# MirceaKitsune/python_raytracer

Measured on AMD Instinct MI355X. Metric: Mrays/s (primary+bounce), higher is better.
Workload: dtype f64; 1 GPU; mods/default 3840x2160 spp8 max_bounces8 (BASELINE config 3/4); width=3840, height=2160, samples=8, primary_rays=62725130, bounce_rays=75192856, partition=(x ^ y) % 1, traversed=True, fast_draws=32, frames_in_flight=1, scene_flow=pre-selected camera chunks (fixture), rng_retraced_rays=0, rng_table=static seeds: draw table + ray table built once before the timed region, reused

## Files before the change

### python_raytracer_amd/csrc/vrt_kernels.hip

```cpp
#include <hip/hip_runtime.h>
#include <stdint.h>
#include <stdio.h>
#include <stdlib.h>

#include <mutex>
#include <vector>

#include "../../include/vrt.h"
#include "vrt_math.h"

#pragma clang fp contract(off)

#define VRT_WAVE 64
#define VRT_BLOCK 256

static thread_local int g_last_hip_error = 0;
#define HIP_TRY(expr)                                   \
    do {                                                \
        hipError_t e__ = (expr);                        \
        if (e__ != hipSuccess) {                        \
            g_last_hip_error = (int)e__;                \
            return VRT_ERR_HIP;                         \
        }                                               \
    } while (0)
// ... 711 lines not shown
    unsigned long long* vals;
    unsigned long long* gkeys;
    unsigned long long* gvals;
};
__device__ __forceinline__ unsigned pow_hash(unsigned long long bits) {
    unsigned h = (unsigned)(bits >> 32) * 0x9e3779b1u + (unsigned)bits * 0x85ebca6bu;
    return h >> 24;
}
#define VRT_PW_PROBES 4
#ifndef VRT_POW_INLINE
#define VRT_POW_INLINE __noinline__
#endif
__device__ VRT_POW_INLINE double pow_miss(unsigned long long* keys, unsigned long long* vals, unsigned long long* gkeys,
                                        unsigned long long* gvals, double x, double y) {
    const double v = vrt_pow(x, y);
    const unsigned long long bits = (unsigned long long)__double_as_longlong(x);
    const unsigned long long vb = (unsigned long long)__double_as_longlong(v);
    const unsigned h = pow_hash(bits);
    for (int i = 0; i < VRT_PW_PROBES; i++) {
        const int s = (int)((h + i) & (VRT_PW_SLOTS - 1));
        const unsigned long long old = atomicCAS(&keys[s], 0ull, bits);
        if (old == 0ull || old == bits) {
            __hip_atomic_store(&vals[s], vb, __ATOMIC_RELAXED, __HIP_MEMORY_SCOPE_WORKGROUP);
            break;
        }
    }
    if (gkeys) {
        for (int i = 0; i < VRT_PW_PROBES; i++) {
            const int s = (int)((h + i) & (VRT_PW_SLOTS - 1));
            const unsigned long long old = atomicCAS(&gkeys[s], 0ull, bits);
            if (old == 0ull || old == bits) {
                __hip_atomic_store(&gvals[s], vb, __ATOMIC_RELAXED, __HIP_MEMORY_SCOPE_AGENT);
                break;
            }
        }
    }
    return v;
}
__device__ VRT_POW_INLINE double pow_slow(unsigned long long* keys, unsigned long long* vals, unsigned long long* gkeys,
                                        unsigned long long* gvals, double x, double y) {
    const unsigned long long bits = (unsigned long long)__double_as_longlong(x);
    const unsigned h = pow_hash(bits);
    for (int i = 1; i < VRT_PW_PROBES; i++) {
        const int sidx = (int)((h + i) & (VRT_PW_SLOTS - 1));
        const unsigned long long k = __hip_atomic_load(&keys[sidx], __ATOMIC_RELAXED, __HIP_MEMORY_SCOPE_WORKGROUP);
        if (k == bits) {
            const unsigned long long v = __hip_atomic_load(&vals[sidx], __ATOMIC_RELAXED, __HIP_MEMORY_SCOPE_WORKGROUP);
            if (v != 0ull) return __longlong_as_double((long long)v);
            break;
        }
        if (k == 0ull) break;
    }
    return pow_miss(keys, vals, gkeys, gvals, x, y);
}
__device__ __forceinline__ double pow_cached(const PowCache& pc, double x, double y) {
    if (x == 1.0) return 1.0;
    const unsigned long long bits = (unsigned long long)__double_as_longlong(x);
    const int sidx = (int)pow_hash(bits);
    const unsigned long long k = __hip_atomic_load(&pc.keys[sidx], __ATOMIC_RELAXED, __HIP_MEMORY_SCOPE_WORKGROUP);
    const unsigned long long v = __hip_atomic_load(&pc.vals[sidx], __ATOMIC_RELAXED, __HIP_MEMORY_SCOPE_WORKGROUP);
    if (k == bits && v != 0ull) return __longlong_as_double((long long)v);
    return pow_slow(pc.keys, pc.vals, pc.gkeys, pc.gvals, x, y);
}

__device__ __forceinline__ bool div_safe(double a) {
    const double m = __builtin_fabs(a);
    return m >= 0x1p-500 && m <= 0x1p500;
}
__device__ __forceinline__ double with_sign_of(double mag, double sgn) {
    const unsigned hi = ((unsigned)__double2hiint(mag) & 0x7fffffffu) | ((unsigned)__double2hiint(sgn) & 0x80000000u);
    return __hiloint2double((int)hi, __double2loint(mag));
}
__device__ __forceinline__ void div3_same_divisor(double& a, double& b, double& c, double d) {
    const bool fast = div_safe(d) & ((a == 0.0) | (__builtin_fabs(a) >= 0x1p-500)) & ((b == 0.0) | (__builtin_fabs(b) >= 0x1p-500)) &
                      ((c == 0.0) | (__builtin_fabs(c) >= 0x1p-500));
    if (fast) {
        double y = __builtin_amdgcn_rcp(d);
        double e = __builtin_fma(-d, y, 1.0);
        y = __builtin_fma(y, e, y);
        e = __builtin_fma(-d, y, 1.0);
        y = __builtin_fma(y, e, y);
        double q, r;
        q = a * y; r = __builtin_fma(-d, q, a); a = with_sign_of(__builtin_fma(r, y, q), a);
        q = b * y; r = __builtin_fma(-d, q, b); b = with_sign_of(__builtin_fma(r, y, q), b);
        q = c * y; r = __builtin_fma(-d, q, c); c = with_sign_of(__builtin_fma(r, y, q), c);
    } else {
        a = a / d;
        b = b / d;
        c = c / d;
    }
}

struct Ray {
    double px, py, pz, vx, vy, vz;
    double step, life, bounces, energy;
    int nm4x, nm4y, nm4z;
    uint32_t entry;
    uint32_t boff;
    uint32_t color;
    int ndraw, resnaps;
    uint32_t off;
    uint32_t rowi;
    double d0, d1, d2;
};

__device__ __forceinline__ unsigned long long wave_first_u64(unsigned long long v) {
    const unsigned lo = __builtin_amdgcn_readfirstlane((unsigned)v), hi = __builtin_amdgcn_readfirstlane((unsigned)(v >> 32));
    return ((unsigned long long)hi << 32) | lo;
}

enum { LANE_IDLE = 0, LANE_MARCH = 1, LANE_HIT = 2, LANE_ENDED = 3, LANE_ENDED_BROKE = 4, LANE_ENDED_EXHAUSTED = 5 };
__device__ __forceinline__ int opaque_zero() {
    int z = 0;
    asm volatile("" : "+v"(z));
    return z;
}
enum { COLD_POS = 0, COLD_ROT = 3, COLD_DIST_MIN = 7, COLD_POW_Y, COLD_LOD_BOUNCES, COLD_MAX_LIGHT, COLD_MAX_BOUNCES1,
       COLD_SHUTTER, COLD_CS, COLD_INV_CS, COLD_N };
enum { C_LOOKUP = 0, C_NBR, C_CGET, C_HIT, C_ADV, C_NLOCAL };

typedef __attribute__((address_space(3))) uint32_t lds_u32;
typedef __attribute__((address_space(3))) double lds_f64;
typedef __attribute__((address_space(3))) unsigned long long lds_u64;
typedef __attribute__((address_space(3))) char lds_char;

struct MarchCtx {
    const lds_char* tab;
    int tl[3];
    const lds_u32* ct;
    lds_u32* bm;
    const lds_f64* mats;
    const lds_f64* cold;
    lds_u32* tot;
    PowCache pc;
    __amdgpu_buffer_rsrc_t vox;
    unsigned cs4;
    double cs, inv_cs;
    bool kept_cs;
    bool has_bm, tile;

    int td[3];
    int toc[3], oc[3], dm[3];
    const lds_char* wt;
    int wb[3];
    unsigned cs3;
};
#define COLD(i) C.cold[(i) + opaque_zero()]
enum { CF_HAS_BM = 1, CF_CT_LDS = 2, CF_CT_IDENTITY = 4, CF_HAS_KEYS = 8, CF_BM_WINDOW = 16 };

#ifdef VRT_DIAG
enum { DG_PASSES = 0, DG_CYC_REFILL, DG_CYC_MARCH, DG_CYC_HIT, DG_CYC_END, DG_ITERS, DG_MARCH_LANES, DG_HIT_EXEC,
       DG_HIT_LANES, DG_END_EXEC, DG_END_LANES, DG_REFILL_EXEC, DG_REFILL_LANES, DG_WAVE_CYCLES, DG_SNAP_ITERS,
       DG_SNAP_LANES, DG_BRICK_VISITS, DG_SWAPS, DG_SWAP_LANES, DG_EVICT_LANES, DG_CYC_SWAP, DG_VOID_LANES,
#ifdef VRT_DIAG_HIST
       DG_NV1, DG_H1 = DG_NV1 + 8, DG_N = DG_H1 + 8
#else
       DG_N
#endif
};
__device__ unsigned long long g_diag[DG_N];
__device__ unsigned long long g_diag_t[5];
#define DG_ADD(idx_, val_)                                                                                      \
    do {                                                                                                        \
        const unsigned long long v_ = (unsigned long long)(val_);   \
        const unsigned long long e_ = __ballot(1);                                                              \
        if ((int)(threadIdx.x & 63) == __ffsll((long long)e_) - 1) dg.acc[idx_] += v_;                           \
    } while (0)
#define DG_TIME() __builtin_amdgcn_s_memtime()
struct DgLane {
    __attribute__((address_space(3))) unsigned long long* acc;
    unsigned brick;
    unsigned long long bv;
};
#define DG_BRICK()                                                                                                     \
    do {                                                                                                               \
        const unsigned key_ = (((unsigned)(int)__builtin_floor(r.px) >> 3) & 1023u) |                                  \
                              ((((unsigned)(int)__builtin_floor(r.py) >> 3) & 1023u) << 10) |                          \
                              ((((unsigned)(int)__builtin_floor(r.pz) >> 3) & 1023u) << 20);                           \
        dg.bv += key_ != dg.brick ? 1 : 0;                                                                             \
        dg.brick = key_;                                                                                               \
    } while (0)
#else
struct DgLane {};
#define DG_ADD(i, v)
#define DG_BRICK()
#endif
#ifdef VRT_ISA_MARK
#define VRT_MARK(name) asm volatile("; @@" name)
#else
#define VRT_MARK(name)
#endif

__device__ __forceinline__ void floor3_i32(double x, double y, double z, int& fx, int& fy, int& fz) {
    double a, b, c;
    const double magic = 6755399441055744.0;
    asm volatile(
        "s_setreg_imm32_b32 hwreg(HW_REG_MODE, 2, 2), 2\n\t"
        "v_add_f64 %0, %3, %6\n\t"
        "v_add_f64 %1, %4, %6\n\t"
        "v_add_f64 %2, %5, %6\n\t"
        "s_setreg_imm32_b32 hwreg(HW_REG_MODE, 2, 2), 0"
        : "=&v"(a), "=&v"(b), "=&v"(c)
        : "v"(x), "v"(y), "v"(z), "s"(magic));
    fx = __double2loint(a);
    fy = __double2loint(b);
    fz = __double2loint(c);
}

__device__ __forceinline__ double min3_f64(double a, double b, double c) {
    double t;
    asm("v_min_f64 %0, %1, %2" : "=v"(t) : "v"(a), "v"(b));
    asm("v_min_f64 %0, %1, %2" : "=v"(t) : "v"(t), "v"(c));
    return t;
}
__device__ __forceinline__ double absmax3_f64(double a, double b, double c) {
    double t;
    asm("v_max_f64 %0, |%1|, |%2|" : "=v"(t) : "v"(a), "v"(b));
    asm("v_max_f64 %0, %1, |%2|" : "=v"(t) : "v"(t), "v"(c));
    return t;
}

__device__ __forceinline__ void floor3_i32_lane(double x, double y, double z, double magic, int& fx, int& fy, int& fz) {
    double a, b, c;
    asm volatile(
        "s_setreg_imm32_b32 hwreg(HW_REG_MODE, 2, 2), 2\n\t"
        "v_add_f64 %0, %3, %6\n\t"
        "v_add_f64 %1, %4, %6\n\t"
        "v_add_f64 %2, %5, %6\n\t"
        "s_setreg_imm32_b32 hwreg(HW_REG_MODE, 2, 2), 0"
        : "=&v"(a), "=&v"(b), "=&v"(c)
        : "v"(x), "v"(y), "v"(z), "v"(magic));
    fx = __double2loint(a);
    fy = __double2loint(b);
    fz = __double2loint(c);
}

__device__ __forceinline__ uint32_t tab_at(const MarchCtx& C, int axis, unsigned byte_index) {
    return *reinterpret_cast<const lds_u32*>(C.tab + C.tl[axis] + (int)byte_index);
}

template <int RESMODE>
__device__ __forceinline__ unsigned cell_offset(const MarchCtx& C, uint32_t entry, unsigned base, unsigned m4, unsigned cs4, int nm4x,
                                                int nm4y, int nm4z, int l4x, int l4y, int l4z, bool inside, bool valid) {
    if (RESMODE == 2 && entry >= (3u << 24)) {
        const int3 o = snap_generic3((int)(entry >> 24), -(nm4x >> 2), -(nm4y >> 2), -(nm4z >> 2), l4x >> 2, l4y >> 2, l4z >> 2);
        l4x = o.x << 2;
        l4y = o.y << 2;
        l4z = o.z << 2;
        inside = valid && (unsigned)(l4x | l4y | l4z) < cs4;
        m4 = 0x3fcu;
    }
    if (RESMODE == 0) m4 = ~0u;
    const unsigned t = tab_at(C, 0, (unsigned)l4x & m4) | tab_at(C, 1, (unsigned)l4y & m4) | tab_at(C, 2, (unsigned)l4z & m4);
    return inside ? base + t : ~0u;
}

__device__ __forceinline__ uint32_t finish_color(const PowCache& pc, bool has_background, double pow_y, double shutter, uint32_t color,
                                                 double& energy, double bounces, double vy) {
    int cr = (int)(color & 255u), cg = (int)((color >> 8) & 255u), cb = (int)((color >> 16) & 255u);
    if (has_background) {
        double a = 1 / pow_cached(pc, 1 + bounces, pow_y);
        if (!(a < 1)) a = 1;
        const double up = vy > 0 ? vy : 0;
        const double b2 = 1 - a;
        cr = (int)__builtin_rint((double)cr * b2 + 127.0 * a);
        cg = (int)__builtin_rint((double)cg * b2 + (127 + up * 64) * a);
        cb = (int)__builtin_rint((double)cb * b2 + (127 + up * 128) * a);
        energy = energy * b2 + (1 + up) * a;
        double t;
        t = __builtin_rint((double)cr * energy); cr = t < 255 ? (int)t : 255;
        t = __builtin_rint((double)cg * energy); cg = t < 255 ? (int)t : 255;
        t = __builtin_rint((double)cb * energy); cb = t < 255 ? (int)t : 255;
    }
    double e = energy + shutter;
    if (!(e < 1)) e = 1;
    const int alpha = (int)__builtin_rint(e * 255);
    return (uint32_t)cr | ((uint32_t)cg << 8) | ((uint32_t)cb << 16) | ((uint32_t)alpha << 24);
}

typedef const __attribute__((address_space(4))) MarchParams* kernarg_ptr;
__device__ __forceinline__ const __attribute__((address_space(4))) MarchParams& fresh_args(const MarchParams&) {
    auto p = (kernarg_ptr)__builtin_amdgcn_kernarg_segment_ptr();
    asm volatile("" : "+s"(p));
    return *p;
}


struct LkState {
    uint32_t okey;
    uint64_t oword;
    uint64_t* brick_slot;
};
template <bool RECORD>
struct SeenList {
    int64_t seen[RECORD ? 48 : 1];
    int n;
};

struct PendingVisit {
    int tci;
    int bi;
    uint64_t tkey, tcur;
};

template <bool RECORD, bool TDQ = false, int DEFER = 0, class PT>
__device__ __forceinline__ void resnap_commit(const PT& Q, const MarchCtx& C, Ray& r, int fx, int fy, int fz, uint64_t wmin_key,
// ... 1176 lines not shown
__device__ __forceinline__ uint32_t morton_even_bits(uint32_t v) {
    v &= 0x55555555u;
    v = (v | (v >> 1)) & 0x33333333u;
    v = (v | (v >> 2)) & 0x0f0f0f0fu;
    v = (v | (v >> 4)) & 0x00ff00ffu;
    v = (v | (v >> 8)) & 0x0000ffffu;
    return v;
}
template <class PT>
__device__ __forceinline__ bool tile_ticket(const PT& Q, uint32_t g, int64_t& first_ray) {
    const uint32_t t = g >> Q.tile_px_log2, c = g & ((1u << Q.tile_px_log2) - 1u);
    const uint32_t tx = morton_even_bits(t), ty = morton_even_bits(t >> 1);
    const uint32_t x = (tx << Q.tile_px_log2) + c;
    first_ray = ((int64_t)x * Q.st.height + (int64_t)(ty << Q.tile_px_log2)) * Q.g.smax;
    return x < (uint32_t)Q.st.width && ty < (uint32_t)Q.tile_nty;
}
__device__ __forceinline__ int tile_take(const MarchParams& P, int ts, int lane, int64_t chunk, int64_t& first_ray) {
    const auto& Q = fresh_args(P);
    const uint32_t per_head = 1u << (Q.tile_px_log2 + 2 * Q.tile_log2 - 3);
    first_ray = -1;
    while ((ts & 0x78) != 0x40) {
        uint32_t k = 0;
        if (lane == 0) k = atomicAdd(Q.tile_heads + (ts & 7) * 32, 1u);
        k = (uint32_t)__builtin_amdgcn_readfirstlane((int)k);
        if (k >= per_head) {
            ts = ((ts + 1) & 7) | ((ts & 0x78) + 8) | 0x80;
            continue;
        }
        if ((int64_t)(per_head - k) * chunk < (int64_t)(gridDim.x >> 3) * (2 * VRT_BLOCK)) ts |= 0x80;
        int64_t first;
        if (tile_ticket(Q, (uint32_t)(ts & 7) * per_head + k, first)) {
            first_ray = first;
            break;
        }
    }
    return ts;
}
#define VRT_POOL_STATE_WORD (13 * 2 * VRT_POOL_SLOTS + 9 * VRT_POOL_SLOTS)
#define VRT_POOL_OFF_WORD (13 * 2 * VRT_POOL_SLOTS + 7 * VRT_POOL_SLOTS)

template <int SPEC, int RESMODE, int PERPIX = 0, bool W = false, bool DEFER = false, bool TILE = false>
__global__ void __launch_bounds__(VRT_BLOCK, VRT_WAVES_PER_SIMD) march_pool_kernel(MarchParams P) {
    static_assert(!TILE || DEFER, "tiled hand-out: the instances for scenes beyond the caches");
    static_assert(!W || (RESMODE != 2 && SPEC == 8), "march_step_w");
    static_assert(!(W && DEFER), "deferred key comparison: the shipped march step");
    __shared__ MarchSharedT<W> S;
    extern __shared__ __align__(16) unsigned char s_dyn[];
    MarchCtx C;
    march_prologue<W>(P, S, s_dyn, C);
    const int wave_in_block = threadIdx.x >> 6;
    const int lane = threadIdx.x & 63;
    lds_u64* const pool = (lds_u64*)(s_dyn + P.pool_lds_off + wave_in_block * VRT_POOL_WAVE_BYTES);
    lds_u32* const pool_state = (lds_u32*)pool + VRT_POOL_STATE_WORD;
    if (lane < VRT_POOL_SLOTS) pool_state[lane] = (uint32_t)LANE_IDLE;
    __syncthreads();

    const int64_t count = P.n;
    const int64_t chunk = P.chunk > 0 ? P.chunk : VRT_CHUNK;
    const int64_t tail_start = count - (int64_t)gridDim.x * (2 * VRT_BLOCK);
    int64_t next = 0, range_end = 0;
    bool more = true;
    bool tiled = false;
    int ts = 0;
    if constexpr (TILE) {
        tiled = P.tile_heads != nullptr && P.plan_hdr->full_frame != 0;
        unsigned xcc = 0;
        xcc = __builtin_amdgcn_s_getreg((3 << 11) | 20);
        ts = (int)(xcc & 7u);
    }

    Ray r;
    r.px = r.py = r.pz = r.vx = r.vy = r.vz = 0;
    r.step = r.life = r.bounces = r.energy = 0;
    r.nm4x = r.nm4y = r.nm4z = 0;
    r.entry = 0;
    r.boff = 0;
    r.color = 0;
    r.ndraw = r.resnaps = 0;
    r.off = 0;
    r.rowi = 0;
    r.d0 = r.d1 = r.d2 = 0.5;
    int state = LANE_IDLE;
    SeenList<false> sl;
    sl.n = 0;
    LkState lk;
    lk.okey = ~0u;
    lk.oword = 0;
    lk.brick_slot = nullptr;
    uint64_t wmin_key = 0;
    DgLane dg;
#ifdef VRT_DIAG
    __shared__ unsigned long long s_dg[VRT_BLOCK / VRT_WAVE][DG_N];
    dg.acc = (__attribute__((address_space(3))) unsigned long long*)&s_dg[threadIdx.x >> 6][0];
    if ((threadIdx.x & 63) == 0)
        for (int j = 0; j < DG_N; j++) dg.acc[j] = 0;
    dg.brick = ~0u;
    dg.bv = 0;
    const unsigned long long dg_t_start = __builtin_amdgcn_s_memrealtime();
    unsigned long long dg_t_empty = 0;
    const unsigned long long dg_start = DG_TIME();
#endif

    auto refill = [&]() {
        unsigned long long idle_mask = __ballot(state == LANE_IDLE);
#ifdef VRT_DIAG
        DG_ADD(DG_REFILL_EXEC, 1);
        DG_ADD(DG_REFILL_LANES, __popcll(idle_mask));
#endif
        while (idle_mask != 0ull && (next < range_end || more)) {
            if (TILE && next >= range_end && tiled) {
                int64_t first = -1;
                ts = tile_take(P, ts, lane, chunk, first);
                if (first < 0) {
                    more = false;
#ifdef VRT_DIAG
                    if (!dg_t_empty) dg_t_empty = __builtin_amdgcn_s_memrealtime();
#endif
                    break;
                }
                next = first;
                range_end = first + chunk;
            } else if (next >= range_end) {
                unsigned long long base = 0;
                if (lane == 0) base = atomicAdd(P.queue_head, (unsigned long long)chunk);
                base = wave_first_u64(base);
                if ((int64_t)base >= count) {
                    more = false;
#ifdef VRT_DIAG
                    if (!dg_t_empty) dg_t_empty = __builtin_amdgcn_s_memrealtime();
#endif
                    break;
                }
                next = (int64_t)base;
                range_end = next + chunk < count ? next + chunk : count;
            }
            const unsigned rank = __builtin_amdgcn_mbcnt_hi((unsigned)(idle_mask >> 32),
                                                            __builtin_amdgcn_mbcnt_lo((unsigned)idle_mask, 0u));
            const int64_t k = next + rank;
            next += __popcll(idle_mask);
            if (state == LANE_IDLE && k < range_end) {
                SeenList<false> none;
                none.n = 0;
                if (take_ray<false, false, PERPIX, W>(P, C, k, r, dg, W ? wmin_key : 0ull, none)) state = LANE_MARCH;
            }
            idle_mask = __ballot(state == LANE_IDLE);
        }
    };
    constexpr bool PASS_COUNTS = W || VRT_PASS_COUNTS;
    int32_t tot[C_NLOCAL];
#pragma unroll
    for (int j = 0; j < C_NLOCAL; j++) tot[j] = 0;
    unsigned pass = 0;
    int stalled = 0;
    for (;; pass++) {
#ifdef VRT_DIAG
        DG_ADD(DG_PASSES, 1);
#endif
        VRT_MARK("pass");
        if (PASS_COUNTS) {
#pragma unroll
            for (int j = 0; j < C_NLOCAL; j++) tot[j] = 0;
        }
        const int sstate = lane < VRT_POOL_SLOTS ? (int)__hip_atomic_load(pool_state + lane, __ATOMIC_RELAXED, __HIP_MEMORY_SCOPE_WAVEFRONT) : -1;
        const bool lane_i = state == LANE_IDLE;
        const unsigned long long l_m = __ballot(state == LANE_MARCH), l_h = __ballot(state == LANE_HIT),
                                 l_e = __ballot(state >= LANE_ENDED), l_i = __ballot(lane_i);
        const unsigned long long s_m = __ballot(sstate == LANE_MARCH), s_h = __ballot(sstate == LANE_HIT),
                                 s_e = __ballot(sstate >= LANE_ENDED), s_f = __ballot(sstate == LANE_IDLE);
        const int n_m = (int)(__popcll(l_m) + __popcll(s_m)), n_h = (int)(__popcll(l_h) + __popcll(s_h)),
                  n_e = (int)(__popcll(l_e) + __popcll(s_e));
        const bool rays_left = next < range_end || more;
        if (stalled > 4096) {
            if (lane == 0) atomicAdd(&S.stats[VRT_S_STALLED], 1ull);
            break;
        }
        const bool evict_ok = rays_left && ((TILE && tiled) ? !(ts & 0x80) : range_end < tail_start);
        const bool can_add = rays_left && (l_i != 0ull || (evict_ok && s_f != 0ull));
        int target;
        if (rays_left) {
            if (n_h >= P.t_hit) target = LANE_HIT;
            else if (n_e >= P.t_end) target = LANE_ENDED;
            else if (n_m > 0 || can_add) target = LANE_MARCH;
            else target = n_h >= n_e ? LANE_HIT : LANE_ENDED;
        } else {
            if (n_m + n_h + n_e == 0) break;
            target = LANE_MARCH;
        }
        const bool tail = !rays_left;
        if (C.has_bm && (pass & 7u) == 0u && (!rays_left || next < range_end)) {
            if (lane == 0) S.wtmp[wave_in_block] = rays_left ? (uint32_t)(P.ray0 + next) : 0xffffffffu;
            if (!lane_i) atomicMin(&S.wtmp[wave_in_block], (uint32_t)(P.ray0 + r.off));
            if (sstate > LANE_IDLE)
                atomicMin(&S.wtmp[wave_in_block],
                          (uint32_t)(P.ray0 + __hip_atomic_load((lds_u32*)pool + VRT_POOL_OFF_WORD + lane, __ATOMIC_RELAXED, __HIP_MEMORY_SCOPE_WAVEFRONT)));
            wmin_key = publish_wave_min(S, wave_in_block, S.wtmp[wave_in_block]);
        }

        VRT_MARK("exchange");
        {
            const bool t_m = target == LANE_MARCH, t_h = target == LANE_HIT;
            const unsigned long long l_t = tail ? ~l_i : (t_m ? l_m : (t_h ? l_h : l_e));
            const unsigned long long c1 = tail ? (s_m | s_h | s_e) : (t_m ? s_m : (t_h ? s_h : s_e));
            const unsigned long long c2 = (t_m && evict_ok) ? s_f : 0ull;
            const unsigned long long l_a = ~(l_t | l_i);
            const int n1 = (int)__popcll(c1), n2 = (int)__popcll(c2), n_a = (int)__popcll(l_a), n_b = (int)__popcll(l_i);
            const int take = n_a + n_b < n1 ? n_a + n_b : n1;
            const int evict = n_a > n1 ? (n_a - n1 < n2 ? n_a - n1 : n2) : 0;
            if (take + evict >= (tail ? 1 : P.pool_swap_min) || (take + evict > 0 && l_t == 0ull)) {
#ifdef VRT_DIAG
                unsigned long long dg_ts = DG_TIME();
                DG_ADD(DG_SWAPS, 1);
                DG_ADD(DG_SWAP_LANES, take + evict);
                DG_ADD(DG_EVICT_LANES, evict);
#endif
                auto rank_in = [&](unsigned long long m) {
                    return (int)__builtin_amdgcn_mbcnt_hi((unsigned)(m >> 32), __builtin_amdgcn_mbcnt_lo((unsigned)m, 0u));
                };
                int crank = 63;
                if (n2 > 0) crank = sel_mask(c2, n1 + rank_in(c2), crank);
                crank = sel_mask(c1, rank_in(c1), crank);
                const int slot_of_rank = __builtin_amdgcn_ds_permute(crank << 2, lane);
                const int brank = sel_mask(l_a, rank_in(l_a), n_a + rank_in(l_i));
                const int my_slot = __builtin_amdgcn_ds_bpermute(brank << 2, slot_of_rank);
                const int limit = sel_mask(l_t, 0, sel_mask(l_a, n1 + n2, n1));
                if (brank < limit) pool_swap(pool, my_slot, P.cs_shift, r, state);
#ifdef VRT_DIAG
                DG_ADD(DG_CYC_SWAP, DG_TIME() - dg_ts);
#endif
            }
        }

        VRT_MARK("select");
        int tv = tail ? 7 : (target == LANE_ENDED ? 1 : (target == LANE_MARCH ? 2 : 4));
        asm volatile("" : "+v"(tv));
#ifdef VRT_DIAG
        unsigned long long dg_t1 = DG_TIME();
        if ((target == LANE_ENDED || tail) && __ballot(state >= LANE_ENDED)) { DG_ADD(DG_END_EXEC, 1); DG_ADD(DG_END_LANES, __popcll(__ballot(state >= LANE_ENDED))); }
#endif
        VRT_MARK("ended");
        if ((tv & 1) && state >= LANE_ENDED) {
            ended_body<false, false>(P, C, r, state, tot, 0, S.stats);
            state = LANE_IDLE;
        }
        VRT_MARK("refill");
#ifdef VRT_DIAG
        unsigned long long dg_t2 = DG_TIME();
        DG_ADD(DG_CYC_END, dg_t2 - dg_t1);
#endif
        if (target != LANE_HIT && (next < range_end || more)) {
            const unsigned long long idle_mask = __ballot(state == LANE_IDLE);
            if (idle_mask != 0ull && (target == LANE_ENDED || (int)__popcll(idle_mask) >= P.pool_refill_min ||
                                      __ballot(state == LANE_MARCH) == 0ull))
                refill();
        }
#ifdef VRT_DIAG
        unsigned long long dg_t3 = DG_TIME();
        DG_ADD(DG_CYC_REFILL, dg_t3 - dg_t2);
#endif
        VRT_MARK("march");
        for (int it = 0; target == LANE_MARCH && it < (tail ? 1 : P.max_iters); it++) {
            const int marching = (int)__popcll(__ballot(state == LANE_MARCH));
            stalled += (it == 0 && marching == 0 && !tail) ? 1 : 0;
            if (marching == 0 || (it > 0 && marching < P.pool_keep)) break;
#ifdef VRT_DIAG
            DG_ADD(DG_ITERS, 1);
            DG_ADD(DG_MARCH_LANES, marching);
#endif
            if (state == LANE_MARCH) {
                if constexpr (W) march_step_w<RESMODE>(P, C, r, state, tot, wmin_key, lk, sl, dg);
                else march_step<SPEC, RESMODE, false, 0, VRT_FRESH_MARCH_POOL, DEFER ? 2 : 0>(P, C, r, state, tot, wmin_key, lk, sl, dg);
            }
        }
#ifdef VRT_DIAG
        unsigned long long dg_t4 = DG_TIME();
        DG_ADD(DG_CYC_MARCH, dg_t4 - dg_t3);
        if ((target == LANE_HIT || tail) && __ballot(state == LANE_HIT)) { DG_ADD(DG_HIT_EXEC, 1); DG_ADD(DG_HIT_LANES, __popcll(__ballot(state == LANE_HIT))); }
#endif
        VRT_MARK("hit");
        if ((tv & 4) && state == LANE_HIT) hit_body<RESMODE, false>(P, C, r, state, tot, dg);
        VRT_MARK("pass_end");
        if (PASS_COUNTS) {
            lds_u32* col = C.tot + (lane & (VRT_TOT_COLS - 1));
            const bool ran_march = tail || target == LANE_MARCH, ran_hit = tail || target == LANE_HIT;
            if (ran_hit) {
                __hip_atomic_fetch_add(col + VRT_C_NBR * VRT_TOT_COLS, (uint32_t)tot[C_NBR], __ATOMIC_RELAXED, __HIP_MEMORY_SCOPE_WORKGROUP);
                __hip_atomic_fetch_add(col + VRT_C_CHUNK_GET * VRT_TOT_COLS, (uint32_t)tot[C_CGET], __ATOMIC_RELAXED, __HIP_MEMORY_SCOPE_WORKGROUP);
                __hip_atomic_fetch_add(col + VRT_C_HIT * VRT_TOT_COLS, (uint32_t)tot[C_HIT], __ATOMIC_RELAXED, __HIP_MEMORY_SCOPE_WORKGROUP);
            }
            if (ran_march) __hip_atomic_fetch_add(col + VRT_C_LOOKUP * VRT_TOT_COLS, (uint32_t)tot[C_LOOKUP], __ATOMIC_RELAXED, __HIP_MEMORY_SCOPE_WORKGROUP);
            if (ran_march || ran_hit) __hip_atomic_fetch_add(col + VRT_C_ADV * VRT_TOT_COLS, (uint32_t)tot[C_ADV], __ATOMIC_RELAXED, __HIP_MEMORY_SCOPE_WORKGROUP);
        }
#ifdef VRT_DIAG
        DG_ADD(DG_CYC_HIT, DG_TIME() - dg_t4);
#endif
    }
    if (!PASS_COUNTS) {
        lds_u32* col = C.tot + (lane & (VRT_TOT_COLS - 1));
        __hip_atomic_fetch_add(col + VRT_C_LOOKUP * VRT_TOT_COLS, (uint32_t)tot[C_LOOKUP], __ATOMIC_RELAXED, __HIP_MEMORY_SCOPE_WORKGROUP);
        __hip_atomic_fetch_add(col + VRT_C_NBR * VRT_TOT_COLS, (uint32_t)tot[C_NBR], __ATOMIC_RELAXED, __HIP_MEMORY_SCOPE_WORKGROUP);
        __hip_atomic_fetch_add(col + VRT_C_CHUNK_GET * VRT_TOT_COLS, (uint32_t)tot[C_CGET], __ATOMIC_RELAXED, __HIP_MEMORY_SCOPE_WORKGROUP);
        __hip_atomic_fetch_add(col + VRT_C_HIT * VRT_TOT_COLS, (uint32_t)tot[C_HIT], __ATOMIC_RELAXED, __HIP_MEMORY_SCOPE_WORKGROUP);
        __hip_atomic_fetch_add(col + VRT_C_ADV * VRT_TOT_COLS, (uint32_t)tot[C_ADV], __ATOMIC_RELAXED, __HIP_MEMORY_SCOPE_WORKGROUP);
    }
#ifdef VRT_DIAG
    diag_flush(dg, dg_start, dg_t_start, dg_t_empty);
#endif
    if (threadIdx.x == 0) atomicAdd(&S.stats[VRT_S_POOL_GROUPS], (TILE && tiled) ? (1ull << 32) + 1ull : 1ull);
    if (W && threadIdx.x == 0) atomicAdd(&S.stats[VRT_S_LOOKAHEAD_GROUPS], 1ull);
    if (PERPIX == 3 && threadIdx.x == 0) atomicAdd(&S.stats[VRT_S_RAYGEN_GROUPS], 1ull);
    march_epilogue<false>(P, S);
}

__device__ __forceinline__ uint32_t resolve_pixel(const vrt_settings& st, int smax, const uint32_t* ray_rgba, int64_t p, int x, int y,
                                                  float4& mean) {
    double dx, dy, det;
    int ns;
    pixel_setup(st, x, y, dx, dy, det, ns);
    uint32_t sr = 0, sg = 0, sb = 0, sa = 0;
    for (int s = 0; s < ns; s++) {
        uint32_t v = ray_rgba[p * smax + s];
        sr += v & 255u;
        sg += (v >> 8) & 255u;
        sb += (v >> 16) & 255u;
        sa += v >> 24;
    }
    const double n = (double)ns;
    const double mr = (double)sr / n, mg = (double)sg / n, mb = (double)sb / n, ma = (double)sa / n;
    mean = make_float4((float)mr, (float)mg, (float)mb, (float)ma);
    return (uint32_t)(unsigned char)(int)mr | ((uint32_t)(unsigned char)(int)mg << 8) | ((uint32_t)(unsigned char)(int)mb << 16) |
           ((uint32_t)(unsigned char)(int)ma << 24);
}
__global__ void __launch_bounds__(VRT_BLOCK) resolve_kernel(vrt_settings st, TileGeom g, const PlanHeader* hdr,
                                                            const uint32_t* ray_rgba, float* rgba_f32, uint8_t* image_u8) {
    __shared__ uint32_t s_tile[16][17];
    if (hdr->full_frame) {
        const int tiles_y = (st.height + 15) / 16;
        const int bx = (int)(blockIdx.x / tiles_y), by = (int)(blockIdx.x % tiles_y);
        if (bx * 16 >= st.width) return;
        const int ty = threadIdx.x & 15, tx = threadIdx.x >> 4;
        const int x = bx * 16 + tx, y = by * 16 + ty;
        if (x < st.width && y < st.height) {
            const int64_t p = (int64_t)x * st.height + y;
            float4 mean;
            const uint32_t px = resolve_pixel(st, g.smax, ray_rgba, p, x, y, mean);
            if (rgba_f32) reinterpret_cast<float4*>(rgba_f32)[p] = mean;
            s_tile[tx][ty] = px;
        }
        __syncthreads();
        if (image_u8) {
            const int wx = threadIdx.x & 15, wy = threadIdx.x >> 4;
            const int ox = bx * 16 + wx, oy = by * 16 + wy;
            if (ox < st.width && oy < st.height) reinterpret_cast<uint32_t*>(image_u8)[(int64_t)oy * st.width + ox] = s_tile[wx][wy];
        }
        return;
    }
    int64_t p = (int64_t)blockIdx.x * VRT_BLOCK + threadIdx.x;
    if (p >= g.n_px) return;
    int x = g.pixels[2 * p], y = g.pixels[2 * p + 1];
    float4 mean;
    const uint32_t px = resolve_pixel(st, g.smax, ray_rgba, p, x, y, mean);
    if (rgba_f32) reinterpret_cast<float4*>(rgba_f32)[p] = mean;
    if (image_u8) reinterpret_cast<uint32_t*>(image_u8)[(int64_t)y * st.width + x] = px;
}

__device__ __forceinline__ void rotate_index(const vrt_object& o, int& x, int& y, int& z) {
    const int ex = o.size[0] - 1, ey = o.size[1] - 1, ez = o.size[2] - 1;
    const int ax = o.turns[0], ay = o.turns[1], az = o.turns[2];
    int a, b, c;
    if (ax && o.size[1] == o.size[2]) {
        a = x;
        b = ax == 1 ? ez - z : (ax == 2 ? ey - y : z);
        c = ax == 1 ? y : (ax == 2 ? ez - z : ey - y);
        x = a, y = b, z = c;
    }
    if (ay && o.size[0] == o.size[2]) {
        a = ay == 1 ? z : (ay == 2 ? ex - x : ez - z);
        b = y;
        c = ay == 1 ? ex - x : (ay == 2 ? ez - z : x);
        x = a, y = b, z = c;
    }
    if (az && o.size[0] == o.size[1]) {
        a = az == 1 ? ey - y : (az == 2 ? ex - x : y);
        b = az == 1 ? x : (az == 2 ? ey - y : ex - x);
        c = z;
        x = a, y = b, z = c;
    }
}

__global__ void __launch_bounds__(VRT_BLOCK) voxelize_kernel(const vrt_object* objects, int n_objects, const uint8_t* models,
                                                             const uint8_t* remap, int ox, int oy, int oz, int dy, int dz,
                                                             int cs, const uint32_t* chunk_list, uint32_t* table, uint8_t* voxels) {
    const int chunk = chunk_list ? (int)chunk_list[blockIdx.x] : (int)blockIdx.x;
    const int cx = chunk / (dy * dz), cy = (chunk / dz) % dy, cz = chunk % dz;
    const int wx0 = ox + cx * cs, wy0 = oy + cy * cs, wz0 = oz + cz * cs;
    uint8_t* block = voxels + (int64_t)chunk * cs * cs * cs;
    int any = 0;
    for (int i = threadIdx.x; i < cs * cs * cs; i += VRT_BLOCK) {
        const int lx = i / (cs * cs), ly = (i / cs) % cs, lz = i % cs;
        const int wx = wx0 + lx, wy = wy0 + ly, wz = wz0 + lz;
        int id = 0;
        for (int k = 0; k < n_objects; k++) {
            const vrt_object& o = objects[k];
            if (wx < o.mins[0] || wy < o.mins[1] || wz < o.mins[2] || wx >= o.maxs[0] || wy >= o.maxs[1] || wz >= o.maxs[2])
                continue;
            int x = wx - o.mins[0], y = wy - o.mins[1], z = wz - o.mins[2];
            rotate_index(o, x, y, z);
            if (x < 0 || y < 0 || z < 0 || x >= o.size[0] || y >= o.size[1] || z >= o.size[2]) continue;
            const int local = models[o.model + ((int64_t)x * o.size[1] + y) * o.size[2] + z];
            if (local) id = remap[o.remap + local];
        }
        block[voxel_offset(cs, lx, ly, lz)] = (uint8_t)id;
        any |= id;
    }
    any = __syncthreads_or(any);
    if (threadIdx.x == 0) table[chunk] = any ? ((uint32_t)(chunk + 1) | (1u << 24)) : 0u;
}

struct SelectParams {
    int32_t origin[3], dims[3];
    int32_t cs, cs_shift, chunk_radius, chunk_lod, culling;
    double cam[3], dist_max;
    int32_t t_origin[3], t_dims[3];
    const unsigned long long* t_keys;
};
__global__ void __launch_bounds__(VRT_BLOCK) select_chunks_kernel(SelectParams S, const uint32_t* world, uint32_t* out) {
    const int64_t n = (int64_t)S.dims[0] * S.dims[1] * S.dims[2];
    const int64_t i = (int64_t)blockIdx.x * VRT_BLOCK + threadIdx.x;
    if (i >= n) return;
    const uint32_t slot = world[i] & 0xffffffu;
    uint32_t e = 0;
    if (slot) {
        const int cz = (int)(i % S.dims[2]), cy = (int)((i / S.dims[2]) % S.dims[1]), cx = (int)(i / ((int64_t)S.dims[2] * S.dims[1]));
        const int px = S.origin[0] + cx * S.cs, py = S.origin[1] + cy * S.cs, pz = S.origin[2] + cz * S.cs;
        bool keep = !S.culling;
        if (!keep && S.t_keys) {
            const int tx = (px - S.t_origin[0]) >> S.cs_shift, ty = (py - S.t_origin[1]) >> S.cs_shift,
                      tz = (pz - S.t_origin[2]) >> S.cs_shift;
            if ((unsigned)tx < (unsigned)S.t_dims[0] && (unsigned)ty < (unsigned)S.t_dims[1] && (unsigned)tz < (unsigned)S.t_dims[2])
                keep = S.t_keys[((int64_t)tx * S.t_dims[1] + ty) * S.t_dims[2] + tz] != ~0ull;
        }
        if (keep) {
            const double dx = (double)(px + S.chunk_radius) - S.cam[0], dy = (double)(py + S.chunk_radius) - S.cam[1],
                         dz = (double)(pz + S.chunk_radius) - S.cam[2];
            const double dist = __builtin_sqrt(dx * dx + dy * dy + dz * dz);
            const double q = __builtin_trunc(dist / (S.dist_max / (double)(1 + S.chunk_lod)));
            const int lod = q < (double)S.chunk_lod ? (int)q : S.chunk_lod;
            e = slot | ((uint32_t)(lod + 1) << 24);
// ... 1216 lines not shown
```

Measured before the change: 26060 Mrays/s.

## Reorder wavefront pass: hit before refill, fall through to march, skip drained pool

Restructures the persistent wavefront pass loop. The hit stage now runs before the end and refill stages. The march loop now runs whatever the chosen target, as long as enough lanes are marching, so lanes that become ready to march are not left idle during hit- or end-target passes. Once no rays are left and the shared pool holds no active slots, the wave enters a drained mode that skips the ballots, target selection and pool exchange. This trims per-pass overhead in the tail, at the cost of changed scheduling order and some extra control divergence.

```diff
diff --git a/python_raytracer_amd/csrc/vrt_kernels.hip b/python_raytracer_amd/csrc/vrt_kernels.hip
--- a/python_raytracer_amd/csrc/vrt_kernels.hip
+++ b/python_raytracer_amd/csrc/vrt_kernels.hip
@@ -887,6 +887,7 @@
 enum { DG_PASSES = 0, DG_CYC_REFILL, DG_CYC_MARCH, DG_CYC_HIT, DG_CYC_END, DG_ITERS, DG_MARCH_LANES, DG_HIT_EXEC,
        DG_HIT_LANES, DG_END_EXEC, DG_END_LANES, DG_REFILL_EXEC, DG_REFILL_LANES, DG_WAVE_CYCLES, DG_SNAP_ITERS,
        DG_SNAP_LANES, DG_BRICK_VISITS, DG_SWAPS, DG_SWAP_LANES, DG_EVICT_LANES, DG_CYC_SWAP, DG_VOID_LANES,
+       DG_FALL_HIT, DG_FALL_END, DG_DRAINED,
 #ifdef VRT_DIAG_HIST
        DG_NV1, DG_H1 = DG_NV1 + 8, DG_N = DG_H1 + 8
 #else
@@ -2369,41 +2370,54 @@
     for (int j = 0; j < C_NLOCAL; j++) tot[j] = 0;
     unsigned pass = 0;
     int stalled = 0;
+    bool drained = false;
     for (;; pass++) {
 #ifdef VRT_DIAG
         DG_ADD(DG_PASSES, 1);
+        if (drained) DG_ADD(DG_DRAINED, 1);
 #endif
         VRT_MARK("pass");
         if (PASS_COUNTS) {
 #pragma unroll
             for (int j = 0; j < C_NLOCAL; j++) tot[j] = 0;
         }
-        const int sstate = lane < VRT_POOL_SLOTS ? (int)__hip_atomic_load(pool_state + lane, __ATOMIC_RELAXED, __HIP_MEMORY_SCOPE_WAVEFRONT) : -1;
+        int sstate = -1;
+        unsigned long long l_m = 0ull, l_h = 0ull, l_e = 0ull, l_i = 0ull, s_m = 0ull, s_h = 0ull, s_e = 0ull, s_f = 0ull;
+        bool rays_left = false, evict_ok = false;
+        int target = LANE_MARCH;
+        if (!drained) {
+            sstate = lane < VRT_POOL_SLOTS ? (int)__hip_atomic_load(pool_state + lane, __ATOMIC_RELAXED, __HIP_MEMORY_SCOPE_WAVEFRONT) : -1;
+            l_m = __ballot(state == LANE_MARCH);
+            l_h = __ballot(state == LANE_HIT);
+            l_e = __ballot(state >= LANE_ENDED);
+            l_i = __ballot(state == LANE_IDLE);
+            s_m = __ballot(sstate == LANE_MARCH);
+            s_h = __ballot(sstate == LANE_HIT);
+            s_e = __ballot(sstate >= LANE_ENDED);
+            s_f = __ballot(sstate == LANE_IDLE);
+            const int n_m = (int)(__popcll(l_m) + __popcll(s_m)), n_h = (int)(__popcll(l_h) + __popcll(s_h)),
+                      n_e = (int)(__popcll(l_e) + __popcll(s_e));
+            rays_left = next < range_end || more;
+            if (stalled > 4096) {
+                if (lane == 0) atomicAdd(&S.stats[VRT_S_STALLED], 1ull);
+                break;
+            }
+            evict_ok = rays_left && ((TILE && tiled) ? !(ts & 0x80) : range_end < tail_start);
+            const bool can_add = rays_left && (l_i != 0ull || (evict_ok && s_f != 0ull));
+            if (rays_left) {
+                if (n_h >= P.t_hit) target = LANE_HIT;
+                else if (n_e >= P.t_end) target = LANE_ENDED;
+                else if (n_m > 0 || can_add) target = LANE_MARCH;
+                else target = n_h >= n_e ? LANE_HIT : LANE_ENDED;
+            } else {
+                if (n_m + n_h + n_e == 0) break;
+                drained = (s_m | s_h | s_e) == 0ull;
+            }
+        } else if (__ballot(state != LANE_IDLE) == 0ull) {
+            break;
+        }
+        const bool tail = !rays_left;
         const bool lane_i = state == LANE_IDLE;
-        const unsigned long long l_m = __ballot(state == LANE_MARCH), l_h = __ballot(state == LANE_HIT),
-                                 l_e = __ballot(state >= LANE_ENDED), l_i = __ballot(lane_i);
-        const unsigned long long s_m = __ballot(sstate == LANE_MARCH), s_h = __ballot(sstate == LANE_HIT),
-                                 s_e = __ballot(sstate >= LANE_ENDED), s_f = __ballot(sstate == LANE_IDLE);
-        const int n_m = (int)(__popcll(l_m) + __popcll(s_m)), n_h = (int)(__popcll(l_h) + __popcll(s_h)),
-                  n_e = (int)(__popcll(l_e) + __popcll(s_e));
-        const bool rays_left = next < range_end || more;
-        if (stalled > 4096) {
-            if (lane == 0) atomicAdd(&S.stats[VRT_S_STALLED], 1ull);
-            break;
-        }
-        const bool evict_ok = rays_left && ((TILE && tiled) ? !(ts & 0x80) : range_end < tail_start);
-        const bool can_add = rays_left && (l_i != 0ull || (evict_ok && s_f != 0ull));
-        int target;
-        if (rays_left) {
-            if (n_h >= P.t_hit) target = LANE_HIT;
-            else if (n_e >= P.t_end) target = LANE_ENDED;
-            else if (n_m > 0 || can_add) target = LANE_MARCH;
-            else target = n_h >= n_e ? LANE_HIT : LANE_ENDED;
-        } else {
-            if (n_m + n_h + n_e == 0) break;
-            target = LANE_MARCH;
-        }
-        const bool tail = !rays_left;
         if (C.has_bm && (pass & 7u) == 0u && (!rays_left || next < range_end)) {
             if (lane == 0) S.wtmp[wave_in_block] = rays_left ? (uint32_t)(P.ray0 + next) : 0xffffffffu;
             if (!lane_i) atomicMin(&S.wtmp[wave_in_block], (uint32_t)(P.ray0 + r.off));
@@ -2414,7 +2428,7 @@
         }
 
         VRT_MARK("exchange");
-        {
+        if (!drained) {
             const bool t_m = target == LANE_MARCH, t_h = target == LANE_HIT;
             const unsigned long long l_t = tail ? ~l_i : (t_m ? l_m : (t_h ? l_h : l_e));
             const unsigned long long c1 = tail ? (s_m | s_h | s_e) : (t_m ? s_m : (t_h ? s_h : s_e));
@@ -2452,6 +2466,13 @@
         asm volatile("" : "+v"(tv));
 #ifdef VRT_DIAG
         unsigned long long dg_t1 = DG_TIME();
+        if ((target == LANE_HIT || tail) && __ballot(state == LANE_HIT)) { DG_ADD(DG_HIT_EXEC, 1); DG_ADD(DG_HIT_LANES, __popcll(__ballot(state == LANE_HIT))); }
+#endif
+        VRT_MARK("hit");
+        if ((tv & 4) && state == LANE_HIT) hit_body<RESMODE, false>(P, C, r, state, tot, dg);
+#ifdef VRT_DIAG
+        unsigned long long dg_t2 = DG_TIME();
+        DG_ADD(DG_CYC_HIT, dg_t2 - dg_t1);
         if ((target == LANE_ENDED || tail) && __ballot(state >= LANE_ENDED)) { DG_ADD(DG_END_EXEC, 1); DG_ADD(DG_END_LANES, __popcll(__ballot(state >= LANE_ENDED))); }
 #endif
         VRT_MARK("ended");
@@ -2461,8 +2482,8 @@
         }
         VRT_MARK("refill");
 #ifdef VRT_DIAG
-        unsigned long long dg_t2 = DG_TIME();
-        DG_ADD(DG_CYC_END, dg_t2 - dg_t1);
+        unsigned long long dg_t3 = DG_TIME();
+        DG_ADD(DG_CYC_END, dg_t3 - dg_t2);
 #endif
         if (target != LANE_HIT && (next < range_end || more)) {
             const unsigned long long idle_mask = __ballot(state == LANE_IDLE);
@@ -2471,34 +2492,34 @@
                 refill();
         }
 #ifdef VRT_DIAG
-        unsigned long long dg_t3 = DG_TIME();
-        DG_ADD(DG_CYC_REFILL, dg_t3 - dg_t2);
+        unsigned long long dg_t4 = DG_TIME();
+        DG_ADD(DG_CYC_REFILL, dg_t4 - dg_t3);
 #endif
         VRT_MARK("march");
-        for (int it = 0; target == LANE_MARCH && it < (tail ? 1 : P.max_iters); it++) {
+        bool marched = false;
+        for (int it = 0; it < (tail ? 1 : P.max_iters); it++) {
             const int marching = (int)__popcll(__ballot(state == LANE_MARCH));
-            stalled += (it == 0 && marching == 0 && !tail) ? 1 : 0;
-            if (marching == 0 || (it > 0 && marching < P.pool_keep)) break;
+            stalled += (it == 0 && marching == 0 && target == LANE_MARCH && !tail) ? 1 : 0;
+            if (marching == 0 || ((it > 0 || target != LANE_MARCH) && marching < P.pool_keep)) break;
 #ifdef VRT_DIAG
+            if (it == 0 && target == LANE_HIT) DG_ADD(DG_FALL_HIT, 1);
+            if (it == 0 && target == LANE_ENDED) DG_ADD(DG_FALL_END, 1);
             DG_ADD(DG_ITERS, 1);
             DG_ADD(DG_MARCH_LANES, marching);
 #endif
+            marched = true;
             if (state == LANE_MARCH) {
                 if constexpr (W) march_step_w<RESMODE>(P, C, r, state, tot, wmin_key, lk, sl, dg);
                 else march_step<SPEC, RESMODE, false, 0, VRT_FRESH_MARCH_POOL, DEFER ? 2 : 0>(P, C, r, state, tot, wmin_key, lk, sl, dg);
             }
         }
 #ifdef VRT_DIAG
-        unsigned long long dg_t4 = DG_TIME();
-        DG_ADD(DG_CYC_MARCH, dg_t4 - dg_t3);
-        if ((target == LANE_HIT || tail) && __ballot(state == LANE_HIT)) { DG_ADD(DG_HIT_EXEC, 1); DG_ADD(DG_HIT_LANES, __popcll(__ballot(state == LANE_HIT))); }
-#endif
-        VRT_MARK("hit");
-        if ((tv & 4) && state == LANE_HIT) hit_body<RESMODE, false>(P, C, r, state, tot, dg);
+        DG_ADD(DG_CYC_MARCH, DG_TIME() - dg_t4);
+#endif
         VRT_MARK("pass_end");
         if (PASS_COUNTS) {
             lds_u32* col = C.tot + (lane & (VRT_TOT_COLS - 1));
-            const bool ran_march = tail || target == LANE_MARCH, ran_hit = tail || target == LANE_HIT;
+            const bool ran_march = marched, ran_hit = tail || target == LANE_HIT;
             if (ran_hit) {
                 __hip_atomic_fetch_add(col + VRT_C_NBR * VRT_TOT_COLS, (uint32_t)tot[C_NBR], __ATOMIC_RELAXED, __HIP_MEMORY_SCOPE_WORKGROUP);
                 __hip_atomic_fetch_add(col + VRT_C_CHUNK_GET * VRT_TOT_COLS, (uint32_t)tot[C_CGET], __ATOMIC_RELAXED, __HIP_MEMORY_SCOPE_WORKGROUP);
@@ -2507,9 +2528,6 @@
             if (ran_march) __hip_atomic_fetch_add(col + VRT_C_LOOKUP * VRT_TOT_COLS, (uint32_t)tot[C_LOOKUP], __ATOMIC_RELAXED, __HIP_MEMORY_SCOPE_WORKGROUP);
             if (ran_march || ran_hit) __hip_atomic_fetch_add(col + VRT_C_ADV * VRT_TOT_COLS, (uint32_t)tot[C_ADV], __ATOMIC_RELAXED, __HIP_MEMORY_SCOPE_WORKGROUP);
         }
-#ifdef VRT_DIAG
-        DG_ADD(DG_CYC_HIT, DG_TIME() - dg_t4);
-#endif
     }
     if (!PASS_COUNTS) {
         lds_u32* col = C.tot + (lane & (VRT_TOT_COLS - 1));
```

Result: faster. 26970 Mrays/s, median of 6 (+3.5%).
